# Picurit/cutter-vad

Measured on AMD Instinct MI355X. Metric: 512-sample frames/sec, Silero V5 16kHz, batch=8192 streams per GPU, higher is better.
Workload: dtype f32

## Files before the change

cutter_vad_amd/csrc/silero_v5_t16_body.h:

```cpp
#define KP(f) k_##f
    using namespace vadk::v5;
    constexpr bool F32IN = FMT == 0;
    constexpr bool G711 = FMT >= 2;
    static_assert(!RS || F32IN, "resampled frames are float32");
    static_assert(!(RS && K8), "the fused resampler feeds the 16 kHz model");
    static_assert(!SCAN || (!RS && !ONE), "a scan is the frame-loop form on audio in HBM");
    static_assert(CH == 1 || (CH == 2 && SCAN), "two interleaved channels: whole recordings only");
    static_assert(!PAIR || (ONE && !RS && !K8 && !G711 && !SCAN), "paired tiles: one-frame calls of the 16 kHz model, float32 / int16");
    constexpr int QL = K8 ? 8 : 16;
    constexpr int CS = 4 * QL;
    constexpr int PP = K8 ? 24 : 48;
    constexpr int LDS_HALF = T_LDS_F4 + (RS ? MT16 * FQ : 0) + (F32IN ? T_FLAG_F4 : 0);
    static_assert(!PAIR || 2 * LDS_HALF * 16 <= 160 * 1024, "both halves' LDS on one CU");
    __shared__ f32x4 lds[(PAIR ? 2 : 1) * LDS_HALF];
    const int hf = PAIR ? __builtin_amdgcn_readfirstlane((int)threadIdx.x >> 8) : 0;
    f32x4 *const ldsH = PAIR ? lds + hf * LDS_HALF : lds;
    [[maybe_unused]] f32x4 *const ldsO = PAIR ? lds + (1 - hf) * LDS_HALF : lds;
    f32x4 *const RX = ldsH;
    [[maybe_unused]] f32x4 *const REV = ldsH + T_EVEN_Q;
    f32x4 *const RE = ldsH + T_ROW_E * QSD;
    f32x4 *const RP0 = ldsH + T_ROW_E0 * QSD;
    f32x4 *const RH = ldsH + T_ROW_H * QSD;
    float *const headp = reinterpret_cast<float *>(RH + T_ROWS_H * QSD);
    float *const nyqv = headp + 64;
// ... 542 lines not shown
                if constexpr (CH == 2) {
                    f32x4 dl, dr;
                    if constexpr (G711) {
                        dl = g711_quad<FMT == 3>(__builtin_amdgcn_perm(b.y, b.x, 0x06040200u));
                        dr = g711_quad<FMT == 3>(__builtin_amdgcn_perm(b.y, b.x, 0x07050301u));
                    } else if constexpr (!f32in) {
                        dl = f32x4{i16_div((int)(short)(b.x & 0xffffu), sc, rsc), i16_div((int)(short)(b.y & 0xffffu), sc, rsc),
                                   i16_div((int)(short)(b.z & 0xffffu), sc, rsc), i16_div((int)(short)(b.w & 0xffffu), sc, rsc)};
                        dr = f32x4{i16_div((int)(short)(b.x >> 16), sc, rsc), i16_div((int)(short)(b.y >> 16), sc, rsc),
                                   i16_div((int)(short)(b.z >> 16), sc, rsc), i16_div((int)(short)(b.w >> 16), sc, rsc)};
                    } else {
                        dl = __builtin_bit_cast(f32x4, u32x4{b.a.x, b.a.z, b.b.x, b.b.z});
                        dr = __builtin_bit_cast(f32x4, u32x4{b.a.y, b.a.w, b.b.y, b.b.w});
                    }
                    const bool right = xmode == 1u, mix = xmode >= 2u;
                    const f32x4 mx = pk::mul(pk::add(dl, dr), f32x4{0.5f, 0.5f, 0.5f, 0.5f});
                    v.x = mix ? mx.x : right ? dr.x : dl.x;
                    v.y = mix ? mx.y : right ? dr.y : dl.y;
                    v.z = mix ? mx.z : right ? dr.z : dl.z;
                    v.w = mix ? mx.w : right ? dr.w : dl.w;
                    if constexpr (f32in) xm = absmax4(xm, v);
                } else if constexpr (G711) {
                    v = g711_quad<FMT == 3>(b);
                } else if constexpr (!f32in) {
                    const int s0 = (int)(short)(b.x & 0xffffu), s1 = (int)(short)(b.x >> 16);
                    const int s2 = (int)(short)(b.y & 0xffffu), s3 = (int)(short)(b.y >> 16);
                    v = f32x4{i16_div(s0, sc, rsc), i16_div(s1, sc, rsc), i16_div(s2, sc, rsc), i16_div(s3, sc, rsc)};
                } else {
                    v = __builtin_bit_cast(f32x4, b);
                    xm = absmax4(xm, v);
                }
                return gate4(v, thr);
            };
#define X_FLAG                                                                                                  \
    if constexpr (f32in) {                                                                                      \
        const unsigned long long b_ = __builtin_amdgcn_ballot_w64(nonfinite(xm));                               \
        flagL[(K8 ? 16 * lcol : 0) + lms] = (uint8_t)(((b_ >> (lane & (64 - QL))) & ((1ull << QL) - 1)) != 0);   \
    }
            auto mirror = [](float v) -> float {
                return __builtin_bit_cast(float, __builtin_amdgcn_mov_dpp(__builtin_bit_cast(int, v), K8 ? 0x141 : 0x140, 0xf, 0xf, true));
            };
            auto shr1 = [&](float edge, float v) -> float {
                const float r = __builtin_bit_cast(float, __builtin_amdgcn_update_dpp(__builtin_bit_cast(int, edge), __builtin_bit_cast(int, v), 0x111, 0xf, 0xf, false));
                return (K8 && q0) ? edge : r;
            };
            auto shl8 = [](float v) -> float {
                return __builtin_bit_cast(float, __builtin_amdgcn_mov_dpp(__builtin_bit_cast(int, v), 0x108, 0xf, 0xf, true));
            };
            [[maybe_unused]] auto ror8hi = [](float lo, float hi) -> float {
                return __builtin_bit_cast(float, __builtin_amdgcn_update_dpp(__builtin_bit_cast(int, lo), __builtin_bit_cast(int, hi), 0x128, 0xf, 0xc, false));
            };
            [[maybe_unused]] const int fold_og = (12 * (q >> 3) + (q & 3)) * QSD + (lms ^ ((q & 3) | ((q >> 3) << 2)));
#define X_FOLD(c, XR, NEXT)                                                                                     \
    {                                                                                                           \
        _Pragma("clang fp contract(off)")                                                                       \
        const int ms = lms;                                                                                     \
        STAMP_ON(20 + (NEXT), XR[3]);                                                                           \
        f32x4 xA, xB;                                                                                           \
        if constexpr (XCARRY && (NEXT)) { xA = xcA; xB = xcB; }                                                 \
        else { xA = decode(XR[0]); xB = decode(XR[1]); }                                                        \
        const f32x4 xC = decode(XR[2]), xD = decode(XR[3]);                                                     \
        if constexpr (XCARRY) { xcA = xC; xcB = xD; }                                                           \
        const float mBx = mirror(xB.x), mDx = mirror(xD.x);                                                     \
        const f32x4 y1 = pk::mul(xA, W1), y3 = pk::mul(xC, W3);                                                 \
        const f32x4 y2 = pk::mul(f32x4{shr1(xC.x, mBx), mirror(xB.w), mirror(xB.z), mirror(xB.y)}, W3);         \
        const f32x4 y4 = pk::mul(f32x4{shr1(0.f, mDx), mirror(xD.w), mirror(xD.z), mirror(xD.y)}, W1);          \
        const f32x4 s14 = pk::add(y1, y4), d14 = pk::sub(y1, y4), s23 = pk::add(y2, y3), d23 = pk::sub(y2, y3); \
        f32x4 pe = pk::add(s14, s23), po = pk::sub(s14, s23), qe = pk::sub(d14, d23), qo = pk::add(d14, d23);   \
        {                                                                                                       \
            pe.x = q0 ? 0.f : pe.x; po.x = q0 ? 0.f : po.x; qe.x = q0 ? 0.f : qe.x; qo.x = q0 ? 0.f : qo.x;        \
            const float y64 = xB.x * w64, y192 = xD.x * w64;                                                    \
            const int fo = q0 ? (c) * 48 + ms : FCOR_SINK + lane;                                               \
            fcor[fo] = y3.x;                                                                                    \
            fcor[fo + (q0 ? 16 : 0)] = y64 + y192;                                                              \
            fcor[fo + (q0 ? 32 : 0)] = y64 - y192;                                                              \
        }                                                                                                       \
        if constexpr (K8) {                                                                                     \
            st2(&RX[(CS * (c) + q) * QSL + ms], pe);                                                            \
            st2(&RX[(CS * (c) + QL + q) * QSL + ms], po);                                                       \
            st2(&RX[(CS * (c) + 2 * QL + q) * QSL + ms], qe);                                                   \
            st2(&RX[(CS * (c) + 3 * QL + q) * QSL + ms], qo);                                                   \
        } else {                                                                                                \
                                                            \
        const f32x4 pm = f32x4{shr1(0.f, mirror(pe.x)), mirror(pe.w), mirror(pe.z), mirror(pe.y)};               \
        const f32x4 qm = f32x4{shr1(0.f, mirror(qe.x)), mirror(qe.w), mirror(qe.z), mirror(qe.y)};               \
        f32x4 pep = pk::add(pe, pm), pen = pk::sub(pe, pm), qen = pk::sub(qe, qm), qep = pk::add(qe, qm);       \
        const float pe32 = shl8(pe.x), qe32 = shl8(qe.x);                                                       \
        pep.x = q0 ? pe32 : pep.x; pen.x = q0 ? 0.f : pen.x; qen.x = q0 ? 0.f : qen.x; qep.x = q0 ? qe32 : qep.x;   \
        f32x4 *const og = RX + (PP * (c)) * QSD + fold_og;                                                      \
        st_planes_half(og, (q >> 2) & 1, po);                                                                   \
        st_planes_half(og + 24 * QSD, (q >> 2) & 1, qo);                                                        \
        const f32x4 eA = f32x4{ror8hi(pep.x, qen.x), ror8hi(pep.y, qen.y), ror8hi(pep.z, qen.z), ror8hi(pep.w, qen.w)};   \
        const f32x4 eB = f32x4{ror8hi(pen.x, qep.x), ror8hi(pen.y, qep.y), ror8hi(pen.z, qep.z), ror8hi(pen.w, qep.w)};   \
        st2(&REV[(32 * (c) + q) * QSL + ms], eA);                                                               \
        st2(&REV[(32 * (c) + 16 + q) * QSL + ms], eB);                                                          \
        }                                                                                                       \
    }
#define H_MIX                                                                                                   \
    _Pragma("unroll") for (int i_ = 0; i_ < 6; ++i_) {                                                          \
        __builtin_amdgcn_sched_group_barrier(0x008, 3, 0);                                                      \
        __builtin_amdgcn_sched_group_barrier(0x002, 28, 0);                                                     \
    }
            if constexpr (RS) H_FIRST(ws_x3, t, true)
            {
                const f32x4 *const bq = biasL + 32 * w + kq;
                if constexpr (PAIR) {
#pragma unroll
                    for (int k = 0; k < 4; ++k) Gp[k][0] = Gp[k][1] = bq[k * 8 + hf * 4];
                } else {
#pragma unroll
                for (int k = 0; k < 8; ++k) G[k] = bq[(k >> 1) * 8 + (k & 1) * 4];
                }
            }
            __syncthreads();
            STAMP(31);
#define H_EXTRA(u)                                                                                              \
            if constexpr (!K8 && (u) + X3_D >= 32) { X3_LDD((u) + X3_D - 32, XU_H + (u) + X3_D) }                \
            if constexpr ((u) == 2 && !RS && !K8) { X_ISSUE(2, xc_, t) }                                        \
            if constexpr ((u) == 15) { if constexpr (K8) { X_FOLD(lcol, xa_, 0) } else { X_FOLD(0, xa_, 0) } H_MIX }   \
            if constexpr ((u) == 23) { if constexpr (K8) { X_FOLD(2, xb_, 1) X_FLAG } else { X_FOLD(1, xb_, 1) } H_MIX }   \
            if constexpr ((u) == 31 && !K8) { X_FOLD(2, xc_, 2) X_FLAG H_MIX }
#define H_FOLDREGION(u) (((u) & 7) >= 5 && (u) >= 8 && ((u) < 24 || !K8))
#define HP_MIX                                                                                                  \
    _Pragma("unroll") for (int i_ = 0; i_ < 6; ++i_) {                                                          \
        __builtin_amdgcn_sched_group_barrier(0x008, 4, 0);                                                      \
        __builtin_amdgcn_sched_group_barrier(0x002, 28, 0);                                                     \
    }
#define HP_EXTRA(v)                                                                                             \
            if constexpr ((v) + X3_D >= 16) { X3_LDD((v) + X3_D - 16, XU_H + (v) + X3_D) }                      \
            if constexpr ((v) == 1) { X_ISSUE(2, xc_, t) }                                                      \
            if constexpr ((v) == 7) { X_FOLD(0, xa_, 0) HP_MIX }                                                \
            if constexpr ((v) == 11) { X_FOLD(1, xb_, 1) HP_MIX }                                               \
            if constexpr ((v) == 15) { X_FOLD(2, xc_, 2) X_FLAG HP_MIX }
#define HP_FOLDREGION(v) (((v) & 3) >= 2 && (v) >= 4)
            if constexpr (PAIR) {
                X3P_HALF(XU_H, wh, RH, (ldsO + T_ROW_H * QSD), HP_EXTRA, HP_FOLDREGION)
            } else {
            X3_HALF(XU_H, wh, RH, H_EXTRA, H_FOLDREGION)
            }
#undef HP_EXTRA
#undef HP_FOLDREGION
#undef HP_MIX
#undef H_EXTRA
#undef H_FOLDREGION
#undef H_MIX
#undef X_FOLD
#undef X_FLAG
        }
        f32x4 Sw[2];
#pragma unroll
        for (int k = 0; k < 2; ++k) Sw[k] = WL(ws_stft + (K8 ? 0 : 8) + k);
        SB();
        STAMP(1);
        __syncthreads();
        STAMP(2);

        {
            const int pair = tid >> 2, pt = tid & 3;
            const int c = pair >> 4, ms = pair & 15;
            float a = 0.f;
            if (pair < 48) {
#pragma unroll
                for (int i = 0; i < 2; ++i) {
                    const f32x4 pp = K8 ? RX[(CS * c + pt * 2 + i) * QSL + ms] : REV[(32 * c + pt * 2 + i) * QSL + ms];
                    a += (pp.x - pp.y) + (pp.z - pp.w);
                }
            }
            a += __shfl_xor(a, 1);
            a += __shfl_xor(a, 2);
            if (pair < 48 && pt == 0) nyqv[c * 16 + ms] = fabsf(a + fcor[(c * 3 + 0) * 16 + ms] + fcor[(c * 3 + 1) * 16 + ms]);
        }

        f32x4 e0f[ENC0_X3_F32_BLOCKS];
#define E0P_BLK(v) (ws_x0 + ENC0_X3_F32_BLOCKS + 3 * (2 * (v) + hf))
#define E0_FIRST                                                                                                \
    _Pragma("unroll") for (int k = 0; k < ENC0_X3_F32_BLOCKS; ++k) e0f[k] = WX(ws_x0 + k);                      \
    _Pragma("unroll") for (int u_ = 0; u_ < X3_D; ++u_) { X3_LDX(ws_x0 + ENC0_X3_F32_BLOCKS + 3 * u_, u_) }
        if constexpr (K8) {
            const bool even = w < 2;
            f32x4 sre[3], sim[3];
#pragma unroll
            for (int c = 0; c < 3; ++c) {
                const float y128 = fcor[(c * 3 + 0) * 16 + n], a64 = fcor[(c * 3 + 1) * 16 + n], b64 = fcor[(c * 3 + 2) * 16 + n];
                const float rp = even ? y128 + a64 : -y128, rm = even ? y128 - a64 : -y128;
                const float ip = even ? 0.f : -b64, im_ = even ? 0.f : b64;
                sre[c] = f32x4{rp, rm, rp, rm};
                sim[c] = f32x4{ip, im_, ip, im_};
            }
            const int rR = even ? 0 : QL, rI = even ? 2 * QL : 3 * QL;
            const f32x4 wr0 = Sw[0], wi0 = Sw[1], wr1 = WL(ws_stft + 2), wi1 = WL(ws_stft + 3);
#pragma unroll
            for (int j = 0; j < 2; ++j) {
                const f32x4 wr = j ? wr1 : wr0, wi = j ? wi1 : wi0;
                f32x4 u[3], v[3];
#pragma unroll
                for (int c = 0; c < 3; ++c) {
                    u[c] = RX[(CS * c + rR + 4 * j) * QSL + nqL];
                    v[c] = RX[(CS * c + rI + 4 * j) * QSL + nqL];
                }
                SB();
#pragma unroll
                for (int c = 0; c < 3; ++c) {
                    sre[c] = mfma16(wr, u[c], sre[c]);
                    sim[c] = mfma16(wi, v[c], sim[c]);
                }
                SB();
            }
            E0_FIRST
            SB();
            __syncthreads();
            {
                f32x4 *o = RX + 12 * (w >> 1) * QSD + nq;
#pragma unroll
                for (int c = 0; c < 3; ++c) st_planes_half(o + PP * c * QSD, w & 1, pk::mag(sre[c], sim[c]));
            }
        } else
        {
            f32x4 are[3][2], aim[3][2];
#pragma unroll
            for (int c = 0; c < 3; ++c) {
                const float y128 = fcor[(c * 3 + 0) * 16 + n], a64 = fcor[(c * 3 + 1) * 16 + n], b64 = fcor[(c * 3 + 2) * 16 + n];
                const float re1 = w < 2 ? y128 - a64 : y128 + a64;
                are[c][0] = f32x4{-y128, -y128, -y128, -y128};
                aim[c][0] = f32x4{-b64, b64, -b64, b64};
                are[c][1] = f32x4{re1, re1, re1, re1};
                aim[c][1] = f32x4{0.f, 0.f, 0.f, 0.f};
            }
            const int nqs[2] = {kq * QSD + (n ^ kq), kq * QSD + (n ^ (kq | 4))};
#define D_RD(c, g, p) __builtin_bit_cast(u32x4, RX[(PP * (c) + 12 * (g) + 4 * (p)) * QSD + nqs[(g) & 1]])
            const int eR = w < 2 ? 16 : 0, eI = w < 2 ? 24 : 8;
            const f32x4 *const XB = REV + nqL;
            f32x4 Aw[2], Bw[2], Au[3], Av[3], Bu[3], Bv[3];
            {
                u32x4 F_[3][3];
#pragma unroll
                for (int c = 0; c < 3; ++c)
#pragma unroll
                    for (int p_ = 0; p_ < 3; ++p_) F_[c][p_] = D_RD(c, 0, p_);
                SB();
                x3_units([&](auto uc_) {
                    constexpr int v_ = decltype(uc_)::value;
                    if constexpr (PAIR) { X3_LDX(E0P_BLK(v_), v_) } else { X3_LDX(ws_x0 + ENC0_X3_F32_BLOCKS + 3 * v_, v_) }
                    if constexpr (v_ == 3) {
#pragma unroll
                        for (int c = 0; c < 3; ++c) { Au[c] = XB[(32 * c + eR) * QSL]; Av[c] = XB[(32 * c + eI) * QSL]; }
                    }
#pragma unroll
                    for (int c = 0; c < 3; ++c) {
                        if constexpr (v_ < 2) are[c][0] = mfma_x3(xw[(XU_D + v_) % X3_NR], F_[c], are[c][0]);
                        else aim[c][0] = mfma_x3(xw[(XU_D + v_) % X3_NR], F_[c], aim[c][0]);
                        if constexpr (v_ + 1 < 4) {
#pragma unroll
                            for (int p_ = 0; p_ < 3; ++p_) F_[c][p_] = D_RD(c, v_ + 1, p_);
                        }
                    }
                    SB();
                }, std::make_integer_sequence<int, 4>{});
            }
#undef D_RD
            if constexpr (PAIR) {
                e0f[0] = WX(ws_x0 + hf);
#pragma unroll
                for (int k = 0; k < 3; ++k) e0f[1 + k] = WX(ws_x0 + 2 + 2 * k + hf);
            } else {
#pragma unroll
                for (int k = 0; k < ENC0_X3_F32_BLOCKS; ++k) e0f[k] = WX(ws_x0 + k);
            }
            SB();
#pragma unroll
            for (int k = 0; k < 2; ++k) Aw[k] = Sw[k];
#define S_LD(S, tt)                                                                        \
    _Pragma("unroll") for (int k = 0; k < 2; ++k) S##w[k] = WL(ws_stft + 2 * (tt) + k);    \
    _Pragma("unroll") for (int c = 0; c < 3; ++c) { S##u[c] = XB[(32 * c + eR + 4 * ((tt) - 4)) * QSL]; S##v[c] = XB[(32 * c + eI + 4 * ((tt) - 4)) * QSL]; }
#define S_MMA(S, rt)                                                                       \
    _Pragma("unroll") for (int j_ = 0; j_ < 4; ++j_)                                       \
        _Pragma("unroll") for (int c = 0; c < 3; ++c) {                                    \
            are[c][rt] = __builtin_amdgcn_mfma_f32_16x16x4f32(S##w[0][j_], S##u[c][j_], are[c][rt], 0, 0, 0); \
            aim[c][rt] = __builtin_amdgcn_mfma_f32_16x16x4f32(S##w[1][j_], S##v[c][j_], aim[c][rt], 0, 0, 0); \
        }
#define S_IL                                                                               \
    __builtin_amdgcn_sched_group_barrier(0x020, 2, 0);                                     \
    _Pragma("unroll") for (int i_ = 0; i_ < 6; ++i_) {                                     \
        __builtin_amdgcn_sched_group_barrier(0x008, 4, 0);                                 \
        __builtin_amdgcn_sched_group_barrier(0x100, 1, 0);                                 \
    }
            S_LD(B, 5) S_MMA(A, 1) S_IL SB();
            S_MMA(B, 1) SB();
#undef S_IL
#undef S_LD
#undef S_MMA
            SB();
            __syncthreads();
#pragma unroll
            for (int c = 0; c < 3; ++c)
                st_planes(RX + (PP * c + 12 * w) * QSD + nq, pk::mag(are[c][0], aim[c][0]), pk::mag(are[c][1], aim[c][1]));
        }
#undef E0_FIRST
        STAMP(3);
        __syncthreads();
        STAMP(4);

        constexpr int NU0 = (K8 ? 2 : 4) * 3 * (PAIR ? 1 : 2);
        f32x4 e1b;
#define E0_EXTRA(u)                                                                                             \
            if constexpr ((u) == NU0 - X3_D) e1b = WY(ws_y1);                                                   \
            if constexpr ((u) + X3_D >= NU0) { X3_LDY(ws_y1 + ENC1_X3_F32_BLOCKS + 3 * ((u) + X3_D - NU0), (u) + X3_D) }
        if constexpr (PAIR) {
            f32x4 acc[3][2];
            const float *const nyqO = reinterpret_cast<const float *>(ldsO + (T_ROW_H + T_ROWS_H) * QSD) + 64;
#pragma unroll
            for (int st = 0; st < 2; ++st) {
                const float *const nq_ = st ? nyqO : nyqv;
                const float nv[3] = {nq_[n], nq_[16 + n], nq_[32 + n]};
#pragma unroll
                for (int o = 0; o < 3; ++o) {
                    f32x4 a = e0f[0];
#pragma unroll
                    for (int t = 0; t < 3; ++t)
                        if (o + t - 1 >= 0 && o + t - 1 < 3) a = pk::fma(e0f[1 + t], pk::splat(nv[o + t - 1]), a);
                    acc[o][st] = a;
                }
            }
#define E0P_SRC(st, c) (((st) ? ldsO : RX) + PP * (c) * QSD)
            u32x4 F_[2][3][3], N1_[2][3];
#pragma unroll
            for (int st = 0; st < 2; ++st)
#pragma unroll
                for (int c_ = 0; c_ < 3; ++c_)
#pragma unroll
                    for (int p_ = 0; p_ < 3; ++p_) F_[st][c_][p_] = PL_RD(E0P_SRC(st, c_), 0, p_);
            SB();
            x3_units([&](auto uc_) {
                constexpr int v_ = decltype(uc_)::value, s_ = v_ / 3, t_ = v_ % 3;
                if constexpr (v_ + X3_D < NU0) { X3_LDX(E0P_BLK(v_ + X3_D), v_ + X3_D) }
                if constexpr (t_ == 1 && s_ + 1 < 4) {
#pragma unroll
                    for (int st = 0; st < 2; ++st)
#pragma unroll
                        for (int p_ = 0; p_ < 3; ++p_) N1_[st][p_] = PL_RD(E0P_SRC(st, 1), s_ + 1, p_);
                }
                E0_EXTRA(v_)
#pragma unroll
                for (int o_ = 0; o_ < 3; ++o_) {
                    const int c_ = o_ + t_ - 1;
                    if (c_ >= 0 && c_ < 3) {
#pragma unroll
                        for (int st = 0; st < 2; ++st) acc[o_][st] = mfma_x3(xw[v_ % X3_NR], F_[st][c_], acc[o_][st]);
                    }
                }
                if constexpr (s_ + 1 < 4 && t_ >= 1) {
#pragma unroll
                    for (int st = 0; st < 2; ++st)
#pragma unroll
                        for (int p_ = 0; p_ < 3; ++p_) {
                            if constexpr (t_ == 1) F_[st][0][p_] = PL_RD(E0P_SRC(st, 0), s_ + 1, p_);
                            else { F_[st][1][p_] = N1_[st][p_]; F_[st][2][p_] = PL_RD(E0P_SRC(st, 2), s_ + 1, p_); }
                        }
                }
                SB();
            }, std::make_integer_sequence<int, NU0>{});
#undef E0P_SRC
#pragma unroll
            for (int st = 0; st < 2; ++st)
#pragma unroll
                for (int c = 0; c < 3; ++c)
                    st_planes_half((st ? ldsO : ldsH) + (T_ROW_E0 + 48 * c + 12 * w) * QSD + nq, hf, relu4(acc[c][st]));
        } else {
            f32x4 acc[3][2];
            {
                const float nv[3] = {nyqv[n], nyqv[16 + n], nyqv[32 + n]};
#pragma unroll
                for (int o = 0; o < 3; ++o)
#pragma unroll
                    for (int rt = 0; rt < 2; ++rt) {
                        f32x4 a = e0f[rt];
#pragma unroll
                        for (int t = 0; t < 3; ++t)
                            if (o + t - 1 >= 0 && o + t - 1 < 3) a = pk::fma(e0f[2 + 2 * t + rt], pk::splat(nv[o + t - 1]), a);
                        acc[o][rt] = a;
                    }
            }
#define E0_SRC(c) (RX + PP * (c) * QSD)
            X3_CONV(K8 ? 2 : 4, 2, 1, 3, X3_LDX, ws_x0 + ENC0_X3_F32_BLOCKS, 0, E0_SRC, acc, E0_EXTRA)
#undef E0_SRC
#pragma unroll
            for (int c = 0; c < 3; ++c) st_planes(RP0 + (48 * c + 12 * w) * QSD + nq, relu4(acc[c][0]), relu4(acc[c][1]));
        }
#undef E0_EXTRA
#undef E0P_BLK
        STAMP(5);
        __syncthreads();
        STAMP(6);

        constexpr int NU1 = 4 * 3, NU2 = 4, NU3 = 4, XU_2 = NU0 + NU1, XU_3 = XU_2 + NU2, XU_L = XU_3 + NU3;
        static_assert(NU2 == X3_D && NU3 == X3_D, "enc1's last X3_D units request enc2's units, enc2's units enc3's, enc3's the input half's first");
        f32x4 e2b, e3b[2];
        {
            f32x4 acc[2][1] = {{e1b}, {e1b}};
#define E1_SRC(c) (RP0 + 48 * (c) * QSD)
#define E1_EXTRA(u)                                                                                             \
            if constexpr ((u) == NU1 - X3_D) {         \
                e2b = WY(ws_z);                                                                                 \
                e3b[0] = WY(ws_z + ENC2_X3_BLOCKS); e3b[1] = WY(ws_z + ENC2_X3_BLOCKS + 1);                     \
            }                                                                                                   \
            if constexpr ((u) + X3_D >= NU1) { X3_LDY(ws_z + 1 + 3 * ((u) + X3_D - NU1), XU_2 + (u) + X3_D - NU1) }
            X3_CONV(4, 1, 2, 2, X3_LDY, ws_y1 + ENC1_X3_F32_BLOCKS, NU0, E1_SRC, acc, E1_EXTRA)
#undef E1_SRC
#undef E1_EXTRA
#pragma unroll
            for (int o = 0; o < 2; ++o) st_planes_half(RX + (24 * o + 12 * (w >> 1)) * QSD + nq, w & 1, relu4(acc[o][0]));
        }
        STAMP(7);
        __syncthreads();
        STAMP(8);

        {
            f32x4 acc = e2b;
            u32x4 F_[2][3];
#pragma unroll
            for (int p_ = 0; p_ < 3; ++p_) F_[0][p_] = PL_RD(RX, 0, p_);
            SB();
            x3_units([&](auto uc_) {
                constexpr int v_ = decltype(uc_)::value;
                X3_LDY(ws_z + ENC2_X3_BLOCKS + 2 + 3 * v_, XU_3 + v_)
                if constexpr (v_ + 1 < NU2) {
#pragma unroll
                    for (int p_ = 0; p_ < 3; ++p_) F_[(v_ + 1) & 1][p_] = PL_RD(RX, v_ + 1, p_);
                }
                acc = mfma_x3(xw[(XU_2 + v_) % X3_NR], F_[v_ & 1], acc);
                SB();
            }, std::make_integer_sequence<int, NU2>{});
            st_planes_half(RE + 12 * (w >> 1) * QSD + nq, w & 1, relu4(acc));
        }
        STAMP(9);
        __syncthreads();
        STAMP(10);

        {
            f32x4 acc[2] = {e3b[0], e3b[1]};
            u32x4 F_[2][3];
#pragma unroll
            for (int p_ = 0; p_ < 3; ++p_) F_[0][p_] = PL_RD(RE, 0, p_);
            SB();
            x3_units([&](auto uc_) {
                constexpr int v_ = decltype(uc_)::value, s_ = v_ >> 1, rt_ = v_ & 1;
                X3_LDU(ws_x3, v_, XU_L)
                if constexpr (v_ == 0) {
#pragma unroll
                    for (int p_ = 0; p_ < 3; ++p_) F_[1][p_] = PL_RD(RE, 1, p_);
                }
                acc[rt_] = mfma_x3(xw[(XU_3 + v_) % X3_NR], F_[s_], acc[rt_]);
                SB();
            }, std::make_integer_sequence<int, NU3>{});
            st_planes(RX + 12 * w * QSD + nq, relu4(acc[0]), relu4(acc[1]));
        }
        STAMP(11);
        __syncthreads();
        STAMP(12);

        {
            const int ws = ws_l + 8;
            f32x4 hw[2];
#define L_EXTRA(u) if constexpr ((u) == 24) { hw[0] = WL(ws + 128); hw[1] = WL(ws + 129); }
#define L_FOLDREGION(u) false
#define LP_EXTRA(v) if constexpr ((v) == 12) { hw[0] = WL(ws + 128); hw[1] = WL(ws + 129); }
            if constexpr (PAIR) {
                X3P_HALF(XU_L, ws_x3, RX, ldsO, LP_EXTRA, L_FOLDREGION)
                f32x4 *const hb = ldsO + (T_ROW_E0 + 16 * w) * QSD + nq;
#pragma unroll
                for (int k = 0; k < 4; ++k) hb[4 * k * QSD] = Gp[k][1];
            } else {
            X3_HALF(XU_L, ws_x3, RX, L_EXTRA, L_FOLDREGION)
            }
#undef LP_EXTRA
#undef L_EXTRA
#undef L_FOLDREGION
            STAMP(18);
            STAMP(13);
            __syncthreads();
            STAMP(14);
            if constexpr (PAIR) {
                const f32x4 *const hb = ldsH + (T_ROW_E0 + 16 * w) * QSD + nq;
#pragma unroll
                for (int k = 0; k < 4; ++k) {
                    const f32x4 o = hb[4 * k * QSD];
                    G[2 * k] = hf ? o : Gp[k][0];
                    G[2 * k + 1] = hf ? Gp[k][0] : o;
                }
            }
            f32x4 part4 = f32x4{0.f, 0.f, 0.f, 0.f};
            const bool rej = f32in && (K8 ? (flagL[n] | flagL[16 + n]) : flagL[n]) != 0;
            const bool bad = SCAN ? (rej || t >= ncol) : rej;
            f32x4 hq[2];
#pragma unroll
            for (int rt = 0; rt < 2; ++rt) {
                const f32x4 i4 = G[0 + rt], f4 = G[2 + rt], g4 = G[4 + rt], o4 = G[6 + rt], c4 = cst[rt], hwv = hw[rt];
                f32x4 cn = pk::fma(pk::sigmoid4(f4), c4, pk::mul(pk::sigmoid4(i4), pk::tanh4(g4)));
                f32x4 hn = pk::mul(pk::sigmoid4(o4), pk::tanh4(cn));
                part4 = pk::fma(hwv, relu4(hn), part4);
                if constexpr ((f32in || SCAN) && !ONE && !RS) {
                    hn = bad ? hv[rt] : hn;
                    cn = bad ? c4 : cn;
                    hv[rt] = hn;
                }
                hq[rt] = hn;
                if (t == T - 1 && live && !((ONE || RS) && bad)) {
                    *reinterpret_cast<f32x4 *>(KP(state) + (size_t)slot * 256 + 32 * w + 16 * rt + 4 * kq) = hn;
                    *reinterpret_cast<f32x4 *>(KP(state) + (size_t)slot * 256 + 128 + 32 * w + 16 * rt + 4 * kq) = cn;
                }
                cst[rt] = cn;
            }
            if constexpr (!ONE && !RS) st_planes(RH + 12 * w * QSD + nq, hq[0], hq[1]);
            float part_ = (part4.x + part4.y) + (part4.z + part4.w);
            part_ += __shfl_xor(part_, 16);
            part_ += __shfl_xor(part_, 32);
            if (kq == 0) headp[w * 16 + n] = part_;
        }
        __syncthreads();
        STAMP(15);

        if (tid < MT16) {
            const float z = hb + ((headp[tid] + headp[16 + tid]) + (headp[32 + tid] + headp[48 + tid]));
            const float p = fminf(sigmoidf_(z), 1.0f);
            if (sm_thread) {
                const bool bad = f32in && (K8 ? (flagL[tid] | flagL[16 + tid]) : flagL[tid]) != 0;
                if constexpr (SCAN) {
                    SmSlot sm = smL[tid];
                    if (t < ncol) {
                        const size_t o = (size_t)obase + (size_t)t;
                        int seg = 0;
                        const int ev = bad ? EV_REJECTED : sm_step(sm, p, &seg);
                        P.probs[o] = bad ? __builtin_nanf("") : p;
                        if (P.events) P.events[o] = (uint8_t)ev;
                        if (P.seg_frames) P.seg_frames[o] = (ev & 2) ? seg : 0;
                    }
                    if (t == T - 1) KP(sm)[sm_slot] = sm;
                    else smL[tid] = sm;
                } else {
                P.probs[(size_t)gf * T + t] = bad ? __builtin_nanf("") : p;
                SmSlot sm = smL[tid];
                int seg = 0;
                const int ev = bad ? EV_REJECTED : sm_step(sm, p, &seg);
                if (t == T - 1) { if (!((ONE || RS) && bad)) KP(sm)[sm_slot] = sm; }
                else smL[tid] = sm;
                if (ev & 2) seg_last = seg;
                if (P.events) P.events[(size_t)gf * T + t] = (uint8_t)ev;
                }
            }
        }
        if (++t >= T) break;
        if constexpr (!RS) H_FIRST(ws_x3, t, true)
    }
#undef H_FIRST
#undef H_FIRSTX
#undef X3_LDU
#undef X3_LDP
#undef X3_LD
#undef X3_LDR
#undef X3_LDX
#undef X3_LDD
#undef X3_LDY
#undef WY
#undef WX
#undef X_ISSUE
#undef X_K0
#undef WL
    if constexpr (!SCAN) { if (sm_thread && P.seg_frames) P.seg_frames[gf] = seg_last; }
    if constexpr (!RS) STAMP(27);
    STAMP_DRAIN(28);
#undef KP
```

Before: 251.5 million.

## Split enc1 and enc3 output channels across paired tile halves

In the paired-tile mode, each half now computes only its share of enc1's and enc3's output channel groups, but for both halves' frames. It reads the partner's LDS activations and writes results into both halves' LDS. This removes duplicated weight-fragment loads and halves the per-half weight unit count for these layers. It also reorders the weight prefetch schedule (enc2 units now prefetch the input half's first units). The cost is more cross-half LDS traffic and tighter coupling between the two halves' synchronisation.

```diff
diff --git a/cutter_vad_amd/csrc/silero_v5_t16_body.h b/cutter_vad_amd/csrc/silero_v5_t16_body.h
--- a/cutter_vad_amd/csrc/silero_v5_t16_body.h
+++ b/cutter_vad_amd/csrc/silero_v5_t16_body.h
@@ -868,9 +868,13 @@
 
         constexpr int NU0 = (K8 ? 2 : 4) * 3 * (PAIR ? 1 : 2);
         f32x4 e1b;
+#define E1P_BLK(v) (ws_y1 + ENC1_X3_F32_BLOCKS + 3 * (3 * ((v) >> 1) + ((v) & 1) + 1 - hf))
 #define E0_EXTRA(u)                                                                                             \
             if constexpr ((u) == NU0 - X3_D) e1b = WY(ws_y1);                                                   \
-            if constexpr ((u) + X3_D >= NU0) { X3_LDY(ws_y1 + ENC1_X3_F32_BLOCKS + 3 * ((u) + X3_D - NU0), (u) + X3_D) }
+            if constexpr ((u) + X3_D >= NU0) {                                                                  \
+                if constexpr (PAIR) { X3_LDY(E1P_BLK((u) + X3_D - NU0), (u) + X3_D) }                           \
+                else { X3_LDY(ws_y1 + ENC1_X3_F32_BLOCKS + 3 * ((u) + X3_D - NU0), (u) + X3_D) }                \
+            }
         if constexpr (PAIR) {
             f32x4 acc[3][2];
             const float *const nyqO = reinterpret_cast<const float *>(ldsO + (T_ROW_H + T_ROWS_H) * QSD) + 64;
@@ -958,10 +962,50 @@
         __syncthreads();
         STAMP(6);
 
-        constexpr int NU1 = 4 * 3, NU2 = 4, NU3 = 4, XU_2 = NU0 + NU1, XU_3 = XU_2 + NU2, XU_L = XU_3 + NU3;
-        static_assert(NU2 == X3_D && NU3 == X3_D, "enc1's last X3_D units request enc2's units, enc2's units enc3's, enc3's the input half's first");
+        constexpr int NU1 = PAIR ? 4 * 2 : 4 * 3, NU2 = 4, NU3 = PAIR ? 2 : 4, XU_2 = NU0 + NU1, XU_3 = XU_2 + NU2, XU_L = XU_3 + NU3;
+        static_assert(NU1 >= X3_D && NU2 == X3_D && (PAIR || NU3 == X3_D),
+                      "enc1's last X3_D units request enc2's units, enc2's units enc3's, enc3's the input half's first");
+        static_assert(!PAIR || (NU3 <= X3_D && NU2 + NU3 >= X3_D),
+                      "paired: enc2's units request enc3's NU3 and the input half's first X3_D - NU3, enc3's the input half's next NU3");
         f32x4 e2b, e3b[2];
-        {
+#define E3_BLK(v) (ws_z + ENC2_X3_BLOCKS + 2 + 3 * (PAIR ? 2 * (v) + hf : (v)))
+        if constexpr (PAIR) {
+            f32x4 acc[2] = {e1b, e1b};
+#define E1P_SRC(st, j) (((st) ? ldsO + T_ROW_E0 * QSD : RP0) + 48 * (hf + (j)) * QSD)
+#define E1_EXTRA(u)                                                                                             \
+            if constexpr ((u) == NU1 - X3_D) {         \
+                e2b = WY(ws_z);                                                                                 \
+                e3b[0] = WY(ws_z + ENC2_X3_BLOCKS + hf);                                \
+            }                                                                                                   \
+            if constexpr ((u) + X3_D >= NU1) { X3_LDY(ws_z + 1 + 3 * ((u) + X3_D - NU1), XU_2 + (u) + X3_D - NU1) }
+            u32x4 F_[2][2][3];
+#pragma unroll
+            for (int st = 0; st < 2; ++st)
+#pragma unroll
+                for (int j_ = 0; j_ < 2; ++j_)
+#pragma unroll
+                    for (int p_ = 0; p_ < 3; ++p_) F_[st][j_][p_] = PL_RD(E1P_SRC(st, j_), 0, p_);
+            SB();
+            x3_units([&](auto uc_) {
+                constexpr int v_ = decltype(uc_)::value, s_ = v_ >> 1, j_ = v_ & 1;
+                if constexpr (v_ + X3_D < NU1) { X3_LDY(E1P_BLK(v_ + X3_D), NU0 + v_ + X3_D) }
+                E1_EXTRA(v_)
+#pragma unroll
+                for (int st = 0; st < 2; ++st) acc[st] = mfma_x3(xw[(NU0 + v_) % X3_NR], F_[st][j_], acc[st]);
+                if constexpr (s_ + 1 < 4) {
+#pragma unroll
+                    for (int st = 0; st < 2; ++st)
+#pragma unroll
+                        for (int p_ = 0; p_ < 3; ++p_) F_[st][j_][p_] = PL_RD(E1P_SRC(st, j_), s_ + 1, p_);
+                }
+                SB();
+            }, std::make_integer_sequence<int, NU1>{});
+#undef E1P_SRC
+#undef E1_EXTRA
+#pragma unroll
+            for (int st = 0; st < 2; ++st)
+                st_planes_half((st ? ldsO : ldsH) + (24 * hf + 12 * (w >> 1)) * QSD + nq, w & 1, relu4(acc[st]));
+        } else {
             f32x4 acc[2][1] = {{e1b}, {e1b}};
 #define E1_SRC(c) (RP0 + 48 * (c) * QSD)
 #define E1_EXTRA(u)                                                                                             \
@@ -976,6 +1020,7 @@
 #pragma unroll
             for (int o = 0; o < 2; ++o) st_planes_half(RX + (24 * o + 12 * (w >> 1)) * QSD + nq, w & 1, relu4(acc[o][0]));
         }
+#undef E1P_BLK
         STAMP(7);
         __syncthreads();
         STAMP(8);
@@ -988,7 +1033,8 @@
             SB();
             x3_units([&](auto uc_) {
                 constexpr int v_ = decltype(uc_)::value;
-                X3_LDY(ws_z + ENC2_X3_BLOCKS + 2 + 3 * v_, XU_3 + v_)
+                if constexpr (v_ < NU3) { X3_LDY(E3_BLK(v_), XU_3 + v_) }
+                else { X3_LDU(ws_x3, v_ - NU3, XU_L) }
                 if constexpr (v_ + 1 < NU2) {
 #pragma unroll
                     for (int p_ = 0; p_ < 3; ++p_) F_[(v_ + 1) & 1][p_] = PL_RD(RX, v_ + 1, p_);
@@ -1002,7 +1048,32 @@
         __syncthreads();
         STAMP(10);
 
-        {
+        if constexpr (PAIR) {
+            f32x4 acc[2] = {e3b[0], e3b[0]};
+#define E3P_SRC(st) ((st) ? ldsO + T_ROW_E * QSD : RE)
+            u32x4 F_[2][2][3];
+#pragma unroll
+            for (int st = 0; st < 2; ++st)
+#pragma unroll
+                for (int p_ = 0; p_ < 3; ++p_) F_[st][0][p_] = PL_RD(E3P_SRC(st), 0, p_);
+            SB();
+            x3_units([&](auto uc_) {
+                constexpr int v_ = decltype(uc_)::value;
+                X3_LDU(ws_x3, v_ + X3_D - NU3, XU_L)
+                if constexpr (v_ == 0) {
+#pragma unroll
+                    for (int st = 0; st < 2; ++st)
+#pragma unroll
+                        for (int p_ = 0; p_ < 3; ++p_) F_[st][1][p_] = PL_RD(E3P_SRC(st), 1, p_);
+                }
+#pragma unroll
+                for (int st = 0; st < 2; ++st) acc[st] = mfma_x3(xw[(XU_3 + v_) % X3_NR], F_[st][v_], acc[st]);
+                SB();
+            }, std::make_integer_sequence<int, NU3>{});
+#undef E3P_SRC
+#pragma unroll
+            for (int st = 0; st < 2; ++st) st_planes_half((st ? ldsO : ldsH) + 12 * w * QSD + nq, hf, relu4(acc[st]));
+        } else {
             f32x4 acc[2] = {e3b[0], e3b[1]};
             u32x4 F_[2][3];
 #pragma unroll
@@ -1020,6 +1091,7 @@
             }, std::make_integer_sequence<int, NU3>{});
             st_planes(RX + 12 * w * QSD + nq, relu4(acc[0]), relu4(acc[1]));
         }
+#undef E3_BLK
         STAMP(11);
         __syncthreads();
         STAMP(12);
```

After: 255.6 million (median of 6 runs). 1.02x the previous value.
